# facebookresearch/hanabi_SAD

Measured on AMD Instinct MI355X. Metric: hanabi_env_steps_per_sec, higher is better.
Workload: dtype u32

## Files before the change

### hanabi_sad_amd/csrc/hsad_env.hip

```cpp

#include <hip/hip_runtime.h>

#include <cstdarg>
#include <cstdlib>
#include <cstdio>
#include <cstring>
#include <new>
#include <string>
#include <vector>

#include "hsad.h"
#include "hsad_deal_fast.h"
#include "hsad_obs_row.h"
#include "hsad_planes.h"

namespace {

constexpr int kWave = 64;
constexpr int kMtN = 624;
constexpr int kMtM = 397;

struct EnvParams {
  static constexpr bool kScripted = false;
  int G, Gpad, P, H, A, F, F0, LAL, OB, OD, OL, OK, DECKW;
  int max_len, sad, shuffle_color, bomb, kmode, n_eps, track_dh, npl;
  int nthreads;
  int gpw;
  int obs_words, legal_words, own_words, win_w;
  int win_words;
  int seed0, deal_mode, nt_stores;
  int g_begin, g_count;
  unsigned long long policy_seed;
  int n_iter;
  int delta;
  int compact;
  int stagger_ticks;
  int stagger_mode;
  int64_t* a_out;
  int64_t* g_out;
  uint32_t* planes;
  uint32_t* mt;
  const float* eps_list;
  uint8_t* deck_hist;
  uint32_t* err;
  uint32_t* act_count;
  unsigned long long* legal_bits;
  float* priv_s;
  float* legal;
  float* own;
  float* eps;
  unsigned long long* priv_bits;
  unsigned long long* legal_out;
  unsigned long long* own_bits;
  unsigned short* priv16;
  int pw64, ld16, obs_f32;
  unsigned dbg_units_hi;
  float* reward;
  uint8_t* terminal;
  unsigned long long* dbg;
  int dbg_iters;
  unsigned dbg_units_lo;
  unsigned long long* phase;
  int part, n_part, lock_ticks;
  unsigned long long launch_tag, first_tag;
  unsigned long long* pace;
  unsigned long long pace_base;
  unsigned long long pace_inv_q32;
  int pace_blocks;
  int pace_l0_q8, pace_cap_ticks;
  int nC, nR, max_info, max_life, deck_max, variant;
  unsigned long long deck_full;
};

struct DealScript {
  uint8_t* cards;
  int32_t* count;
};
struct ScriptedParams : EnvParams {
  static constexpr bool kScripted = true;
  DealScript sc;
};

constexpr uint32_t kIdentityPerm = (0u) | (1u << 3) | (2u << 6) | (3u << 9) | (4u << 12);
constexpr uint32_t kIdentityPermBoth = kIdentityPerm | (kIdentityPerm << 15);
__host__ __device__ constexpr uint64_t full_deck_bits() {
  uint64_t d = 0;
  for (int c = 0; c < 5; ++c) {
    const int cnt[5] = {3, 2, 2, 2, 1};
    for (int r = 0; r < 5; ++r) d |= (uint64_t)cnt[r] << (2 * (c * 5 + r));
  }
  return d;
}

__host__ __device__ constexpr uint64_t deck_bits(int C, int R) {
  uint64_t d = 0;
  for (int c = 0; c < C; ++c)
    for (int r = 0; r < R; ++r) d |= (uint64_t)(r == 0 ? 3 : (r == R - 1 ? 1 : 2)) << (2 * (c * 5 + r));
  return d;
}

struct Rules {
  int C, R, MI, ML;
  int deck;
  uint64_t full;
  uint32_t cmask, rmask;
  int CR, KS, DW;
};
struct FullRules {
  static constexpr int C = 5, R = 5, MI = 8, ML = 3, deck = 50;
  static constexpr uint64_t full = full_deck_bits();
  static constexpr uint32_t cmask = 31u, rmask = 31u;
  static constexpr int CR = 25, KS = 35, DW = 10;
};
template <bool V>
struct RulesOf {
  static __device__ __forceinline__ FullRules make(const EnvParams&) { return FullRules{}; }
};
template <>
struct RulesOf<true> {
  static __device__ __forceinline__ Rules make(const EnvParams& ep) {
    const int C = ep.nC, R = ep.nR;
    return Rules{C, R, ep.max_info, ep.max_life, ep.deck_max, ep.deck_full, (1u << C) - 1u, (1u << R) - 1u, C * R,
                 C * R + C + R, R == 1 ? 3 : 2 * R};
  }
};

constexpr uint32_t kMtUpper = 0x80000000u, kMtLower = 0x7fffffffu, kMtMag = 0x9908b0dfu;

__device__ __forceinline__ uint32_t mt_temper(uint32_t x) {
  x ^= x >> 11;
  x ^= (x << 7) & 0x9d2c5680u;
  x ^= (x << 15) & 0xefc60000u;
  x ^= x >> 18;
  return x;
// ... 903 lines not shown
  return df_select(mask, h % (uint32_t)__popcll(mask));
}
__device__ __forceinline__ uint64_t policy_key(uint64_t seed, uint64_t game, int p, int stream) {
  return mix64(seed ^ mix64(game * 0xD1342543DE82EF95ull + (uint64_t)(p * 2 + stream)));
}
__device__ __forceinline__ int policy_pick_keyed(uint64_t key, uint64_t counter, uint64_t mask, int nbits) {
  const uint32_t h = (uint32_t)(mix64(key + counter) >> 32);
  return df_select(mask, h % (uint32_t)__popcll(mask), nbits);
}

constexpr int kEnvThreads = 4 * kWave;

__device__ __forceinline__ void stream_rows(const EnvParams& ep, const uint32_t* s_obs, const uint32_t* s_legal, const uint32_t* s_own,
                                            int g0, int ng, int P, int H, int t, int n) {
  const size_t PF = (size_t)P * ep.F, PA = (size_t)P * ep.A, PO = (size_t)P * 3 * H;
  if (!ep.obs_f32) {
  } else if (ep.nt_stores) {
    stream_bits_f32_aligned<true>(s_obs, ep.priv_s + (size_t)g0 * PF, (uint32_t)(ng * PF), t, n);
  } else {
    stream_bits_f32_aligned<false>(s_obs, ep.priv_s + (size_t)g0 * PF, (uint32_t)(ng * PF), t, n);
  }
  stream_rows_packed(ep, s_obs, 0, ng * P, (size_t)g0 * P, t, n);
  stream_bits_f32_aligned<false>(s_legal, ep.legal + (size_t)g0 * PA, (uint32_t)(ng * PA), t, n);
  stream_bits_f32_aligned<false>(s_own, ep.own + (size_t)g0 * PO, (uint32_t)(ng * PO), t, n);
}

__device__ __forceinline__ unsigned stream_rows_delta(const EnvParams& ep, const uint32_t* s_obs, uint32_t* s_old, bool all,
                                                      const uint32_t* s_legal, const uint32_t* s_own, int g0, int ng, int P, int H,
                                                      int t, int n, bool count, int compact, unsigned& units) {
  const size_t PF = (size_t)P * ep.F, PA = (size_t)P * ep.A, PO = (size_t)P * 3 * H;
  unsigned stored = 0;
  bool by_lines = true;
  if (!ep.obs_f32) {
  } else if (compact && !all) {
    by_lines = false;
    float* out = ep.priv_s + (size_t)g0 * PF;
    if (compact == 2) {
      if (ep.nt_stores) {
        stored = stream_bits_f32_compact<true, 16>(s_obs, s_old, out, (uint32_t)(ng * PF), t, units);
      } else {
        stored = stream_bits_f32_compact<false, 16>(s_obs, s_old, out, (uint32_t)(ng * PF), t, units);
      }
    } else if (ep.nt_stores) {
      stored = stream_bits_f32_compact<true, 32>(s_obs, s_old, out, (uint32_t)(ng * PF), t, units);
    } else {
      stored = stream_bits_f32_compact<false, 32>(s_obs, s_old, out, (uint32_t)(ng * PF), t, units);
    }
  } else if (ep.nt_stores) {
    stored = stream_bits_f32_delta<true>(s_obs, s_old, all, ep.priv_s + (size_t)g0 * PF, (uint32_t)(ng * PF), t, n, count);
  } else {
    stored = stream_bits_f32_delta<false>(s_obs, s_old, all, ep.priv_s + (size_t)g0 * PF, (uint32_t)(ng * PF), t, n, count);
  }
  if (by_lines) units = stored;
  stream_rows_packed(ep, s_obs, 0, ng * P, (size_t)g0 * P, t, n);
  stream_bits_f32_aligned<false>(s_legal, ep.legal + (size_t)g0 * PA, (uint32_t)(ng * PA), t, n);
  stream_bits_f32_aligned<false>(s_own, ep.own + (size_t)g0 * PO, (uint32_t)(ng * PO), t, n);
  return stored;
}

__device__ __forceinline__ void clear_words(uint32_t* p, int nz, int t, int n) {
  uint4* z4 = reinterpret_cast<uint4*>(p);
  for (int k = t; k < (nz >> 2); k += n) z4[k] = make_uint4(0u, 0u, 0u, 0u);
  for (int k = (nz & ~3) + t; k < nz; k += n) p[k] = 0u;
}

__device__ __forceinline__ void clear_rows(const EnvParams& ep, uint32_t* s_obs, int t, int n) {
  const int nz = ep.obs_words + ep.legal_words + ep.own_words;
  uint4* z4 = reinterpret_cast<uint4*>(s_obs);
  for (int k = t; k < (nz >> 2); k += n) z4[k] = make_uint4(0u, 0u, 0u, 0u);
  for (int k = (nz & ~3) + t; k < nz; k += n) s_obs[k] = 0u;
}

struct LogicCarry {
  uint32_t* counter;
  const uint32_t* s_lmask;
  const uint64_t* pkey;
};
template <int TP, int TH>
constexpr bool kPolicyKeys = (TP == 2 && TH == 5);
template <int N>
__device__ __forceinline__ uint64_t carried_key(const uint64_t* k, int i) {
  uint64_t v = k[0];
#pragma unroll
  for (int j = 1; j < N; ++j) v = (i == j) ? k[j] : v;
  return v;
}
typedef __attribute__((address_space(3))) const uint32_t* LdsWordPtr;

template <int MODE, int TP, int TH, bool V = false, class EP = EnvParams, bool CARRY = false>
__device__ __forceinline__ void env_logic(const EP& ep, const int64_t* __restrict__ a_in, const int64_t* __restrict__ g_in,
                                          uint32_t* s_st, uint32_t* s_win, const float* s_eps, const int lane, const int g,
                                          const bool active, const bool do_reset, Rng& rng, uint32_t& greedy_rec, float& reward,
                                          bool& term, const int dbg_it = 0, const LogicCarry carry = {nullptr, nullptr, nullptr}) {
  const int P = TP ? TP : ep.P, H = TH ? TH : ep.H;
  const auto ru = RulesOf<V>::make(ep);
  if (MODE == 0 || MODE == 3) {
    const int W = ep.win_w;
    constexpr int kWmin = (TP && !V) ? (2 * TP * TH + TP + 2 < 64 ? 2 * TP * TH + TP + 2 : 64) : 0;
    constexpr int kWmax = (TP && !V) ? (kWmin + 1 + 2 * (TP - 1) < 64 ? kWmin + 1 + 2 * (TP - 1) : 64) : 64;
    constexpr int kNB = kWmax <= 32 ? kWmax : 32;
    uint32_t* winA = s_win + lane;
    uint32_t* winB = s_win + (W <= 32 ? 0 : (W + 1) * kWave) + lane;
    const uint32_t wbase = rng.spos;
    if (do_reset) {
      if (kWmax <= 32 || (kWmin <= 32 && W <= 32)) {
        const uint32_t* pw = rng.mt + wbase;
// ... 375 lines not shown
        __builtin_amdgcn_s_sleep(8);
      }
    }
  }
  STAMP_START();
  const uint32_t misc0 = ep.planes[(size_t)PL_MISC * ep.Gpad + g];
  bool active;
  const bool needs_reset = valid && (!((misc0 >> 15) & 1u) || ((misc0 >> 14) & 1u));
  if (MODE == 0) {
    active = needs_reset;
    if (__ballot(active) == 0ull) return;
  } else {
    active = valid;
  }
  const bool do_reset = (MODE == 0 || MODE == 3) && needs_reset;
  if (wave == 0) {
    for (int pl0 = 0; pl0 < ep.npl; pl0 += 8) {
      uint32_t v[8];
#pragma unroll
      for (int j = 0; j < 8; ++j) v[j] = ep.planes[(size_t)min(pl0 + j, ep.npl - 1) * ep.Gpad + g];
#pragma unroll
      for (int j = 0; j < 8; ++j)
        if (pl0 + j < ep.npl) ST(pl0 + j) = v[j];
    }
  } else {
    const int zt = tid - kWave, zn = nthreads - kWave;
    clear_rows(ep, s_obs, zt, zn);
    if (MODE == 0 || MODE == 3)
      for (int k = zt; k < min(ep.n_eps, 128); k += zn) s_eps[k] = ep.eps_list[k];
  }
  __syncthreads();
  STAMP(1);

  Rng rng;
  rng.mt = ep.mt + (size_t)g * kMtN;
  rng.draws = ST(PL_DRAWS);
  rng.la0 = ST(PL_LA0);
  rng.la1 = ST(PL_LA1);
  rng.la_n = (int)((ST(PL_MISC) >> 22) & 3u);
  rng.spos = (rng.draws + (uint32_t)rng.la_n) % (uint32_t)kMtN;
  rng.win = nullptr;
  rng.w_c = rng.w_n = 0;
  uint32_t greedy_rec = 0;
  float reward = 0.f;
  bool term = false;

  if (wave == 0) {
    env_logic<MODE, TP, TH, V>(ep, a_in, g_in, s_st, s_win, s_eps, lane, g, active, do_reset, rng, greedy_rec, reward, term, dbg_it);
    s_grec[lane] = greedy_rec;
  }
  __syncthreads();
  STAMP(2);

  Refill rf;
  refill_issue(rf, rng, active && wave == 0);
  if (active) build_rows<TP, TH, V>(ep, s_st, lane, g, s_obs, s_legal, s_own, s_grec[lane], wave, nwaves);
  STAMP(3);
  if (active && wave == 0) {
    refill_finish(rf, rng);
    ST(PL_DRAWS) = rng.draws;
    ST(PL_LA0) = rng.la0;
    ST(PL_LA1) = rng.la1;
    ST(PL_MISC) = (ST(PL_MISC) & ~(3u << 22)) | ((uint32_t)rng.la_n << 22);
    for (int pl = 0; pl < ep.npl; ++pl) ep.planes[(size_t)pl * ep.Gpad + g] = ST(pl);
  }
  __syncthreads();
  STAMP(4);

  const size_t PF = (size_t)P * ep.F, PA = (size_t)P * ep.A, PO = (size_t)P * 3 * H;
  if (MODE >= 1) {
    stream_rows(ep, s_obs, s_legal, s_own, g0, ng, P, H, tid, nthreads);
    if (valid && wave == 0) {
      for (int p = 0; p < P; ++p) ep.eps[(size_t)g * P + p] = __uint_as_float(ST(PLEPS(p)));
      ep.reward[g] = reward;
      ep.terminal[g] = term ? 1 : 0;
    }
    if (ep.kmode == 1) {
      __syncthreads();
      if (wave == 0) v0_fixup<V>(ep, s_st, s_obs, __ballot(valid), g0, lane);
    }
  } else {
    if (wave != 0) return;
    uint64_t todo = __ballot(active);
    const uint64_t todo_all = todo;
    while (todo) {
      const int lg = __builtin_ctzll(todo);
      todo &= todo - 1;
      if (ep.obs_f32) stream_bits_f32(s_obs, (uint32_t)(lg * PF), ep.priv_s + (size_t)(g0 + lg) * PF, (uint32_t)PF, lane);
      stream_rows_packed(ep, s_obs, lg * P, P, (size_t)(g0 + lg) * P, lane, kWave);
      stream_bits_f32(s_legal, (uint32_t)(lg * PA), ep.legal + (size_t)(g0 + lg) * PA, (uint32_t)PA, lane);
      stream_bits_f32(s_own, (uint32_t)(lg * PO), ep.own + (size_t)(g0 + lg) * PO, (uint32_t)PO, lane);
    }
    if (active)
      for (int p = 0; p < P; ++p) ep.eps[(size_t)g * P + p] = __uint_as_float(ST(PLEPS(p)));
    if (ep.kmode == 1) {
      __syncthreads();
      v0_fixup<V>(ep, s_st, s_obs, todo_all, g0, lane);
    }
  }
  STAMP(5);
}

template <int MODE, int TP, int TH, bool V = false>
__global__ __launch_bounds__(kEnvThreads) void env_kernel(EnvParams ep, const int64_t* __restrict__ a_in,
                                                          const int64_t* __restrict__ g_in) {
  env_body<MODE, TP, TH, V>(ep, a_in, g_in);
}

template <int TP, int TH, bool V = false>
__global__ __launch_bounds__(kEnvThreads) void env_step_scripted_kernel(ScriptedParams ep, const int64_t* __restrict__ a_in,
                                                                        const int64_t* __restrict__ g_in) {
  env_body<1, TP, TH, V>(ep, a_in, g_in);
}

__device__ __forceinline__ void rollout_stagger(const EnvParams& ep) {
  if (ep.stagger_ticks > 0) {
    unsigned k = blockIdx.x & 7u;
    if (ep.stagger_mode == 1) k = ((blockIdx.x >> 3) >> 5) & 3u;
    else if (ep.stagger_mode == 2) k = (blockIdx.x >> 3) & 3u;
    else if (ep.stagger_mode == 3) {
      unsigned hw;
      asm volatile("s_getreg_b32 %0, hwreg(HW_REG_HW_ID)" : "=s"(hw));
      k = (hw & 15u) >> 1;
    }
// ... 1 lines not shown
    while (wall_clock64() - t_in < wait) __builtin_amdgcn_s_sleep(16);
  }
}

__device__ __forceinline__ unsigned pace_delay(const EnvParams& ep, unsigned long long s, int iter, unsigned t_own) {
  const long long num = (long long)iter * ep.pace_blocks - (long long)(s - ep.pace_base);
  const long long span = (long long)ep.n_iter * ep.pace_blocks;
  if (num < -span || num > span) return 0u;
  const int over_q8 = (int)((num * (long long)ep.pace_inv_q32) >> 24) - ep.pace_l0_q8;
  if (over_q8 <= 0) return 0u;
  t_own = min(t_own, 1u << 20);
  const unsigned long long d = ((unsigned long long)(unsigned)over_q8 * t_own) >> 8;
  return (unsigned)min(d, (unsigned long long)min(t_own >> 1, (unsigned)ep.pace_cap_ticks));
}

__device__ __forceinline__ unsigned long long pace_count(const EnvParams& ep) {
  int z = 0;
  unsigned long long one = 1ull;
  asm volatile("" : "+v"(z), "+v"(one));
  return __hip_atomic_fetch_add(ep.pace + z, one, __ATOMIC_RELAXED, __HIP_MEMORY_SCOPE_AGENT);
}

__device__ __forceinline__ void pace_sleep(unsigned ticks) {
  const unsigned long long t_in = wall_clock64();
  while (wall_clock64() - t_in < (unsigned long long)ticks) __builtin_amdgcn_s_sleep(16);
}

template <int TP, int TH, bool V = false>
__global__ __launch_bounds__(kEnvThreads) __attribute__((amdgpu_waves_per_eu(2, 2))) void env_rollout_kernel(EnvParams ep) {
  rollout_stagger(ep);
  unsigned long long pace_s = 0ull;
  unsigned pace_t0 = (unsigned)wall_clock64();
  const bool paced = ep.pace && ep.g_begin + (int)blockIdx.x * ep.gpw < ep.G;
#pragma clang loop unroll(disable)
  for (int iter = 0; iter < ep.n_iter; ++iter) {
    if (iter) __syncthreads();
    if (paced) {
      const unsigned now = (unsigned)wall_clock64(), t_own = now - pace_t0;
      pace_t0 = now;
      if (threadIdx.x == 0) {
        if (iter > 0) {
          const unsigned d = pace_delay(ep, pace_s, iter - 1, t_own);
          if (d) pace_sleep(d);
        }
        pace_s = pace_count(ep);
      }
    }
    int zero = 0;
    asm volatile("" : "+s"(zero));
    env_body<3, TP, TH, V>(ep, nullptr, nullptr, zero, iter);
  }
}

#ifdef HSAD_ENV_ROWBUILD_SCATTER
template <int TP, int TH>
constexpr bool kRowBuildFixed = false;
#else
template <int TP, int TH>
constexpr bool kRowBuildFixed = TP > 0 && TH > 0;
#endif

__device__ __forceinline__ unsigned wave_sum(unsigned v) {
  for (int o = kWave / 2; o > 0; o >>= 1) v += (unsigned)__shfl_xor((int)v, o, kWave);
  return v;
}

constexpr int kChainIn = 2, kChainOut = 4;
constexpr int kPrioShift = 3;
__device__ __forceinline__ uint4* chain_slice(const EnvParams& ep) {
  return reinterpret_cast<uint4*>(reinterpret_cast<uint32_t*>(ep.phase) + (size_t)blockIdx.x * ep.obs_words);
}

template <int TP, int TH>
__global__ __launch_bounds__(kEnvThreads) __attribute__((amdgpu_waves_per_eu(2, 2))) void env_rollout_pipe_kernel(EnvParams ep) {
  if constexpr (kRowBuildFixed<TP, TH>) asm volatile("" ::: "v175");
  rollout_stagger(ep);
  extern __shared__ __attribute__((aligned(16))) uint32_t smem[];
  uint32_t* s_st = smem;
  uint32_t* s_obs = s_st + ep.npl * kWave;
  uint32_t* s_legal = s_obs + ep.obs_words;
  uint32_t* s_own = s_legal + ep.legal_words;
  uint32_t* s_win = s_own + ep.own_words;
  uint32_t* s_grec = s_win + ep.win_words * kWave;
  float* s_eps = reinterpret_cast<float*>(s_grec + kWave);
  uint32_t* s_pace = s_grec + kWave + 128;
#define S_OBS1(z) (delta ? s_pace + 4 + (z) : s_obs)
  const int delta = ep.delta & 7;

  const int tid = threadIdx.x;
  const int lane = tid & (kWave - 1);
  const int wave = tid >> 6;
  const int g0 = ep.g_begin + blockIdx.x * ep.gpw;
  const int ng = min(ep.gpw, ep.G - g0);
  if (ng <= 0) return;
  const int P = TP ? TP : ep.P, H = TH ? TH : ep.H;

  unsigned hw_self;
  asm volatile("s_getreg_b32 %0, hwreg(HW_REG_HW_ID)" : "=s"(hw_self));
  const int prio_mode = (ep.delta >> kPrioShift) & 3;
  const int prio_role = (prio_mode & 2) ? 2 * __builtin_amdgcn_readfirstlane(wave) : 0;
  const int prio_alt = prio_mode & 1, prio_slot = (int)(hw_self & 15u);

  uint32_t act_counter = 0u;
  uint64_t pkey[kPolicyKeys<TP, TH> ? 2 * TP : 1] = {};
  if (wave == 0) {
    const int g = g0 + lane;
    if (lane < ng) {
      act_counter = ep.act_count[g];
      if constexpr (kPolicyKeys<TP, TH>) {
#pragma unroll
        for (int k = 0; k < 2 * TP; ++k) pkey[k] = policy_key(ep.policy_seed, (uint64_t)g, k >> 1, k & 1);
      }
      for (int p = 0; p < P; ++p) {
        const uint64_t lm = ep.legal_bits[(size_t)g * P + p];
        s_win[(2 * p) * kWave + lane] = (uint32_t)lm;
        s_win[(2 * p + 1) * kWave + lane] = (uint32_t)(lm >> 32);
      }
    }
    for (int pl0 = 0; pl0 < ep.npl; pl0 += 8) {
      uint32_t v[8];
// ... 356 lines not shown
  size_t d_records_cap;
  uint8_t* d_log_script;
  int32_t* d_log_count;
  int64_t* d_log_a;
};

namespace {

typedef void (*EnvKernelFn)(EnvParams, const int64_t*, const int64_t*);

EnvKernelFn pick_env_kernel(int mode, int P, int H, bool variant) {
  if (variant) {
    switch (mode) {
      case 0: return env_kernel<0, 0, 0, true>;
      case 1: return env_kernel<1, 0, 0, true>;
      case 2: return env_kernel<2, 0, 0, true>;
      default: return env_kernel<3, 0, 0, true>;
    }
  }
#define HSAD_ENV_SPECIALISE(PP, HH)                 \
  if (P == PP && H == HH) {                         \
    switch (mode) {                                 \
      case 0: return env_kernel<0, PP, HH>;         \
      case 1: return env_kernel<1, PP, HH>;         \
      case 2: return env_kernel<2, PP, HH>;         \
      default: return env_kernel<3, PP, HH>;        \
    }                                               \
  }
  HSAD_ENV_SPECIALISE(2, 5)
  HSAD_ENV_SPECIALISE(5, 4)
  HSAD_ENV_SPECIALISE(3, 5)
  HSAD_ENV_SPECIALISE(4, 4)
#undef HSAD_ENV_SPECIALISE
  switch (mode) {
    case 0: return env_kernel<0, 0, 0>;
    case 1: return env_kernel<1, 0, 0>;
    case 2: return env_kernel<2, 0, 0>;
    default: return env_kernel<3, 0, 0>;
  }
}

typedef void (*EnvScriptedStepFn)(ScriptedParams, const int64_t*, const int64_t*);
EnvScriptedStepFn pick_scripted_step_kernel(int P, int H, bool variant) {
  if (variant) return env_step_scripted_kernel<0, 0, true>;
  if (P == 2 && H == 5) return env_step_scripted_kernel<2, 5>;
  if (P == 5 && H == 4) return env_step_scripted_kernel<5, 4>;
  if (P == 3 && H == 5) return env_step_scripted_kernel<3, 5>;
  if (P == 4 && H == 4) return env_step_scripted_kernel<4, 4>;
  return env_step_scripted_kernel<0, 0>;
}

typedef void (*EnvRolloutFn)(EnvParams);
constexpr int kRolloutPrioDefault = 2;
constexpr int kPaceL0Q8 = 0;
constexpr int kPaceCapTicks = 3500;
bool rollout_pipelined(const hsad_env* e) {
  return e->rollout_pipe && e->ep.nthreads == 2 * kWave && e->ep.kmode == 0 && !e->ep.variant;
}

bool rollout_delta_active(const hsad_env* e) {
  return e->rollout_delta && e->delta_fits && rollout_pipelined(e) && e->ep.obs_f32;
}

bool rollout_paced(const hsad_env* e) {
  if (e->rollout_pace >= 0) return e->rollout_pace != 0;
  return !(e->rollout_compact && rollout_delta_active(e));
}

int rollout_chain_mode(const hsad_env* e) {
  return rollout_delta_active(e) && !e->chain_unavailable ? e->rollout_chain : 0;
}

EnvRolloutFn pick_rollout_kernel(int P, int H, bool pipe, bool variant) {
  if (variant) return env_rollout_kernel<0, 0, true>;
#define HSAD_ROLLOUT_SPECIALISE(PP, HH) \
  if (P == PP && H == HH) return pipe ? env_rollout_pipe_kernel<PP, HH> : env_rollout_kernel<PP, HH>;
  HSAD_ROLLOUT_SPECIALISE(2, 5)
  HSAD_ROLLOUT_SPECIALISE(5, 4)
  HSAD_ROLLOUT_SPECIALISE(3, 5)
  HSAD_ROLLOUT_SPECIALISE(4, 4)
#undef HSAD_ROLLOUT_SPECIALISE
  return pipe ? env_rollout_pipe_kernel<0, 0> : env_rollout_kernel<0, 0>;
}

int configure_env_kernels(hsad_env* e) {
  HIP_TRY(hipFuncSetAttribute(reinterpret_cast<const void*>(pick_rollout_kernel(e->ep.P, e->ep.H, false, e->ep.variant != 0)),
                              hipFuncAttributeMaxDynamicSharedMemorySize, (int)e->lds_bytes_reset));
  e->delta_fits = false;
  if (!e->ep.variant) {
    const void* fn = reinterpret_cast<const void*>(pick_rollout_kernel(e->ep.P, e->ep.H, true, false));
    const bool room = e->lds_bytes_delta <= 160 * 1024;
    HIP_TRY(hipFuncSetAttribute(fn, hipFuncAttributeMaxDynamicSharedMemorySize, (int)(room ? e->lds_bytes_delta : e->lds_bytes_reset)));
    if (room) {
      int wg_full = 0, wg_delta = 0;
      HIP_TRY(hipOccupancyMaxActiveBlocksPerMultiprocessor(&wg_full, fn, 2 * kWave, e->lds_bytes_reset));
      HIP_TRY(hipOccupancyMaxActiveBlocksPerMultiprocessor(&wg_delta, fn, 2 * kWave, e->lds_bytes_delta));
      e->delta_fits = wg_delta >= 1 && wg_delta >= wg_full;
    }
  }
  for (int mode = 0; mode < 4; ++mode) {
    const size_t lds = (mode == 1 || mode == 2) ? e->lds_bytes : e->lds_bytes_reset;
    HIP_TRY(hipFuncSetAttribute(reinterpret_cast<const void*>(pick_env_kernel(mode, e->ep.P, e->ep.H, e->ep.variant != 0)),
                                hipFuncAttributeMaxDynamicSharedMemorySize, (int)lds));
  }
  return HSAD_OK;
}

void launch_env(hsad_env* e, int mode, const int64_t* a, const int64_t* g, hipStream_t stream, int g_begin,
                int g_count, uint64_t policy_seed = 0, int64_t* a_out = nullptr, int64_t* g_out = nullptr, int part = -1,
                unsigned long long tag = 0, unsigned long long first_tag = 0, int n_part = 1, int n_iter = 1,
                int chain = 0) {
  size_t lds = (mode == 1 || mode == 2) ? e->lds_bytes : e->lds_bytes_reset;
  EnvParams ep = e->ep;
  ep.delta = mode == 3 && n_iter > 1 && rollout_delta_active(e) ? 1 : 0;
  ep.compact = ep.delta && e->rollout_compact ? (e->rollout_unit == 64 ? 2 : 1) : 0;
  if (ep.delta) lds = e->lds_bytes_delta;
  ep.phase = part >= 0 ? e->d_phase : nullptr;
  ep.part = part < 0 ? 0 : part;
  ep.lock_ticks = (int)(e->stagger_ns / 10);
  ep.launch_tag = tag;
  ep.first_tag = first_tag;
  if (part < 0 && ep.delta && chain && e->d_chain) {
    ep.phase = reinterpret_cast<unsigned long long*>(e->d_chain);
    ep.delta |= chain;
  }
  if (mode == 3 && n_iter > 1 && rollout_pipelined(e)) ep.delta |= e->rollout_prio << kPrioShift;
  ep.n_part = n_part;
  ep.g_begin = g_begin;
  ep.g_count = g_count;
  ep.policy_seed = policy_seed;
  ep.n_iter = n_iter;
  ep.stagger_ticks = n_iter > 1 ? (int)(e->stagger_ns / 10) : 0;
  static const int stagger_mode = getenv("HSAD_ENV_STAGGER_MODE") ? atoi(getenv("HSAD_ENV_STAGGER_MODE")) : 0;
  ep.stagger_mode = stagger_mode;
  ep.a_out = a_out;
  ep.g_out = g_out;
  ep.pace = nullptr;
  if (mode == 3 && n_iter > 1 && rollout_paced(e)) {
    const int g_end = std::min(ep.G, g_begin + g_count);
    const long long blocks = g_end > g_begin ? (g_end - g_begin + ep.gpw - 1) / ep.gpw : 0;
    if (blocks > 0 && blocks * n_iter < (1ll << 29)) {
      ep.pace = e->d_pace;
      ep.pace_base = e->pace_base + (unsigned long long)e->pace_bias;
      ep.pace_blocks = (int)blocks;
      ep.pace_inv_q32 = (1ull << 32) / (unsigned long long)blocks;
      ep.pace_l0_q8 = e->pace_l0_q8;
      ep.pace_cap_ticks = e->pace_cap_ticks;
      e->pace_base += (unsigned long long)(blocks * n_iter);
    }
  }
  if (mode == 3 && n_iter > 1)
    hipLaunchKernelGGL(pick_rollout_kernel(ep.P, ep.H, rollout_pipelined(e), ep.variant != 0), dim3((g_count + ep.gpw - 1) / ep.gpw), dim3(ep.nthreads), lds, stream, ep);
  else if (mode == 1 && e->scripted) {
    ScriptedParams sp;
    static_cast<EnvParams&>(sp) = ep;
    sp.sc = e->script;
    hipLaunchKernelGGL(pick_scripted_step_kernel(ep.P, ep.H, ep.variant != 0), dim3((g_count + ep.gpw - 1) / ep.gpw), dim3(ep.nthreads),
                       lds, stream, sp, a, g);
  }
  else
    hipLaunchKernelGGL(pick_env_kernel(mode, ep.P, ep.H, ep.variant != 0), dim3((g_count + ep.gpw - 1) / ep.gpw), dim3(ep.nthreads), lds,
                       stream, ep, a, g);
}

}

extern "C" {

const char* hsad_last_error(void) { return g_last_error.c_str(); }
int hsad_internal_set_error(int code, const char* msg) {
  g_last_error = msg ? msg : "";
  return code;
}
const char* hsad_version(void) { return "hsad 0.1 gfx950"; }

int hsad_env_create(const hsad_env_config* cfg, hsad_env** out) { return hsad_env_create_rules(cfg, nullptr, out); }

int hsad_env_create_rules(const hsad_env_config* cfg, const hsad_env_rules* rules, hsad_env** out) {
  if (!cfg || !out) return set_error(HSAD_ERR_INVALID, "null argument");
  *out = nullptr;
  const hsad_env_rules full = {5, 5, 8, 3};
  const hsad_env_rules ru = rules ? *rules : full;
  if (ru.colors < 1 || ru.colors > 5) return set_error(HSAD_ERR_INVALID, "colors must be 1..5");
  if (ru.ranks < 1 || ru.ranks > 5) return set_error(HSAD_ERR_INVALID, "ranks must be 1..5");
  if (ru.max_information_tokens < 1 || ru.max_information_tokens > 8)
    return set_error(HSAD_ERR_INVALID, "max_information_tokens must be 1..8");
  if (ru.max_life_tokens < 1 || ru.max_life_tokens > 3) return set_error(HSAD_ERR_INVALID, "max_life_tokens must be 1..3");
  const int Cn = ru.colors, Rn = ru.ranks;
  const int deck_max = Cn * (Rn == 1 ? 3 : 2 * Rn);
  if (cfg->num_games < 1) return set_error(HSAD_ERR_INVALID, "num_games must be >= 1");
  if (cfg->players < 2 || cfg->players > 5) return set_error(HSAD_ERR_INVALID, "players must be 2..5");
  if (cfg->hand_size < 1 || cfg->hand_size > 5) return set_error(HSAD_ERR_INVALID, "hand_size must be 1..5");
  if (cfg->players * cfg->hand_size > deck_max)
    return set_error(HSAD_ERR_INVALID, "players * hand_size (%d) exceeds the deck (%d cards)", cfg->players * cfg->hand_size, deck_max);
  if (cfg->shuffle_obs) return set_error(HSAD_ERR_INVALID, "shuffle_obs is not supported (reference asserts it off)");
  if (cfg->n_eps < 1 || !cfg->eps_list) return set_error(HSAD_ERR_INVALID, "eps_list must hold >= 1 value");
  if (cfg->knowledge_mode != 0 && cfg->knowledge_mode != 1) return set_error(HSAD_ERR_INVALID, "knowledge_mode 0|1");
  if (cfg->max_len > 255) return set_error(HSAD_ERR_INVALID, "max_len must be <= 255");
  if (cfg->games_per_workgroup != 0 && cfg->games_per_workgroup != 32 && cfg->games_per_workgroup != 64)
    return set_error(HSAD_ERR_INVALID, "games_per_workgroup must be 0 (auto), 32 or 64");
  HIP_TRY(hipSetDevice(cfg->device));

  hsad_env* e = new (std::nothrow) hsad_env();
  if (!e) return set_error(HSAD_ERR_NOMEM, "host allocation failed");
// ... 254 lines not shown
}

int hsad_env_step(hsad_env* e, const int64_t* a, const int64_t* greedy_a, void* stream) {
  if (!e) return set_error(HSAD_ERR_INVALID, "null env");
  if (!e->bound) return set_error(HSAD_ERR_STATE, "hsad_env_bind_outputs must be called first");
  if (!a) return set_error(HSAD_ERR_INVALID, "action tensor is null");
  if (e->ep.sad && !greedy_a) return set_error(HSAD_ERR_INVALID, "sad=1 requires greedy_a");
  launch_env(e, 1, a, greedy_a, (hipStream_t)stream, 0, e->ep.Gpad);
  HIP_TRY(hipGetLastError());
  return HSAD_OK;
}

int hsad_env_policy_random(hsad_env* e, uint64_t policy_seed, int64_t* a, int64_t* greedy_a, void* stream) {
  if (!e) return set_error(HSAD_ERR_INVALID, "null env");
  if (!e->bound) return set_error(HSAD_ERR_STATE, "hsad_env_bind_outputs must be called first");
  if (!a) return set_error(HSAD_ERR_INVALID, "action tensor is null");
  EnvParams ep = e->ep;
  ep.g_begin = 0;
  ep.g_count = ep.G;
  hipLaunchKernelGGL(policy_kernel, dim3((ep.G + 255) / 256), dim3(256), 0, (hipStream_t)stream, ep, policy_seed, a,
                     greedy_a);
  HIP_TRY(hipGetLastError());
  return HSAD_OK;
}

int hsad_env_set_partitions(hsad_env* e, int n_part) {
  if (!e) return set_error(HSAD_ERR_INVALID, "null env");
  if (n_part < 1 || n_part > 16) return set_error(HSAD_ERR_INVALID, "n_part must be 1..16");
  const int blocks = e->ep.Gpad / e->ep.gpw;
  if (n_part > blocks) n_part = blocks;
  HIP_TRY(hipSetDevice(e->device));
  for (int k = e->n_part; k < n_part; ++k) {
    HIP_TRY(hipStreamCreateWithFlags(&e->part_stream[k], hipStreamNonBlocking));
    HIP_TRY(hipEventCreate(&e->part_done[k]));
    HIP_TRY(hipEventCreate(&e->part_begin[k]));
  }
  if (!e->fork) HIP_TRY(hipEventCreateWithFlags(&e->fork, hipEventDisableTiming));
  if (n_part > e->n_part) e->n_part = n_part;
  e->n_part_active = n_part;
  return HSAD_OK;
}

int hsad_env_rollout_random(hsad_env* e, int n_iter, uint64_t policy_seed, int64_t* a, int64_t* greedy_a,
                            void* stream) {
  if (!e) return set_error(HSAD_ERR_INVALID, "null env");
  if (!e->bound) return set_error(HSAD_ERR_STATE, "hsad_env_bind_outputs must be called first");
  if (!a) return set_error(HSAD_ERR_INVALID, "action tensor is null");
  if (e->ep.sad && !greedy_a) return set_error(HSAD_ERR_INVALID, "sad=1 requires greedy_a");
  if (e->scripted) return set_error(HSAD_ERR_STATE, "hsad_env_rollout_random: the env holds a deal script (only hsad_env_step deals from it; hsad_env_reset clears it)");
  const int K = e->n_part_active;
  const int blocks = e->ep.Gpad / e->ep.gpw;
  if (e->rollout_chunk > 0) {
    bool chained = rollout_chain_mode(e) != 0 && n_iter > e->rollout_chunk;
    if (chained && !e->d_chain) {
      if (hipMalloc((void**)&e->d_chain, sizeof(uint32_t) * (size_t)blocks * e->ep.obs_words) != hipSuccess) {
        (void)hipGetLastError();
        e->d_chain = nullptr;
        e->chain_unavailable = true;
        chained = false;
      }
    }
    int chain = 0;
    for (int i = 0; i < n_iter; i += e->rollout_chunk) {
      const int n = std::min(e->rollout_chunk, n_iter - i), n_next = std::min(e->rollout_chunk, n_iter - i - n);
      chain = (chain & kChainOut ? kChainIn : 0) | (chained && n > 1 && n_next > 1 ? kChainOut : 0);
      launch_env(e, 3, nullptr, nullptr, (hipStream_t)stream, 0, e->ep.Gpad, policy_seed, a, greedy_a, -1, 0, 0, 1, n, chain);
    }
    HIP_TRY(hipGetLastError());
    return HSAD_OK;
  }
  if (K <= 1) {
    for (int i = 0; i < n_iter; ++i)
      launch_env(e, 3, nullptr, nullptr, (hipStream_t)stream, 0, e->ep.Gpad, policy_seed, a, greedy_a);
    HIP_TRY(hipGetLastError());
    return HSAD_OK;
  }
  HIP_TRY(hipEventRecord(e->fork, (hipStream_t)stream));
  for (int k = 0; k < K; ++k) {
    HIP_TRY(hipStreamWaitEvent(e->part_stream[k], e->fork, 0));
    HIP_TRY(hipEventRecord(e->part_begin[k], e->part_stream[k]));
  }
  e->last_rollout_iters = n_iter;
  e->last_rollout_parts = K;
  if (!e->d_phase) {
    HIP_TRY(hipMalloc((void**)&e->d_phase, sizeof(unsigned long long) * 32));
    HIP_TRY(hipMemset(e->d_phase, 0, sizeof(unsigned long long) * 32));
  }
  const unsigned long long first_tag = e->launch_seq + 1;
  for (int i = 0; i < n_iter; ++i) {
    const unsigned long long tag = ++e->launch_seq;
    for (int k = 0; k < K; ++k) {
      const int b0 = (int)((long long)blocks * k / K), b1 = (int)((long long)blocks * (k + 1) / K);
      if (b1 <= b0) continue;
      launch_env(e, 3, nullptr, nullptr, e->part_stream[k], b0 * e->ep.gpw, (b1 - b0) * e->ep.gpw, policy_seed, a, greedy_a, k, tag,
                 first_tag, K);
    }
  }
  HIP_TRY(hipGetLastError());
  for (int k = 0; k < K; ++k) {
    HIP_TRY(hipEventRecord(e->part_done[k], e->part_stream[k]));
    HIP_TRY(hipStreamWaitEvent((hipStream_t)stream, e->part_done[k], 0));
  }
  return HSAD_OK;
}

int hsad_env_last_rollout_ms(hsad_env* e, float* ms_per_launch, int* n_part) {
  if (!e || !ms_per_launch) return set_error(HSAD_ERR_INVALID, "null argument");
  const int K = e->last_rollout_parts;
  if (n_part) *n_part = K;
  if (K < 2 || e->last_rollout_iters < 1) return set_error(HSAD_ERR_STATE, "no partitioned rollout has run");
  for (int k = 0; k < K; ++k) {
    float ms = 0.f;
    HIP_TRY(hipEventSynchronize(e->part_done[k]));
    HIP_TRY(hipEventElapsedTime(&ms, e->part_begin[k], e->part_done[k]));
    ms_per_launch[k] = ms / (float)e->last_rollout_iters;
  }
  return HSAD_OK;
}

int hsad_env_set_rollout_chunk(hsad_env* e, int iterations_per_launch) {
  if (!e || iterations_per_launch < 0) return set_error(HSAD_ERR_INVALID, "bad argument");
  e->rollout_chunk = iterations_per_launch;
  return HSAD_OK;
}

int hsad_env_set_rollout_pace(hsad_env* e, int on) {
  if (!e) return set_error(HSAD_ERR_INVALID, "null env");
  e->rollout_pace = on != 0;
  return HSAD_OK;
}

int hsad_env_rollout_pace_cap_us(const hsad_env* e) { return e ? e->pace_cap_ticks / 100 : 0; }

int hsad_env_set_rollout_delta(hsad_env* e, int on) {
  if (!e) return set_error(HSAD_ERR_INVALID, "null env");
  e->rollout_delta = on != 0;
  return HSAD_OK;
}

int hsad_env_rollout_delta_active(const hsad_env* e) { return e && rollout_delta_active(e) ? 1 : 0; }

int hsad_env_set_rollout_chain(hsad_env* e, int mode) {
  if (!e || (mode != 0 && mode != 1)) return set_error(HSAD_ERR_INVALID, "the rollout chain mode is 0 or 1");
  e->rollout_chain = mode;
  return HSAD_OK;
}

int hsad_env_rollout_chain_active(const hsad_env* e) { return e ? rollout_chain_mode(e) : 0; }

int hsad_env_set_rollout_prio(hsad_env* e, int mode) {
  if (!e || mode < 0 || mode > 3) return set_error(HSAD_ERR_INVALID, "the rollout priority mode is 0..3");
  e->rollout_prio = mode;
  return HSAD_OK;
}

int hsad_env_rollout_prio(const hsad_env* e) { return e && rollout_pipelined(e) ? e->rollout_prio : 0; }

int hsad_env_set_rollout_compact(hsad_env* e, int on) {
  if (!e) return set_error(HSAD_ERR_INVALID, "null env");
  e->rollout_compact = on != 0;
  return HSAD_OK;
}

int hsad_env_rollout_compact_active(const hsad_env* e) { return e && e->rollout_compact && rollout_delta_active(e) ? 1 : 0; }

int hsad_env_set_rollout_unit(hsad_env* e, int bytes) {
  if (!e || (bytes != 128 && bytes != 64)) return set_error(HSAD_ERR_INVALID, "the rollout unit is 128 or 64 bytes");
  e->rollout_unit = bytes;
  return HSAD_OK;
}

int hsad_env_rollout_unit(const hsad_env* e) { return e ? (hsad_env_rollout_compact_active(e) ? e->rollout_unit : 128) : 0; }

int hsad_env_debug_pace_bias(hsad_env* e, int64_t bias) {
  if (!e) return set_error(HSAD_ERR_INVALID, "null env");
  e->pace_bias = (long long)bias;
  return HSAD_OK;
}

int hsad_env_debug_pace_word(hsad_env* e, int64_t* device_word, int64_t* host_base) {
  if (!e || !device_word || !host_base) return set_error(HSAD_ERR_INVALID, "null argument");
  unsigned long long w = 0;
  HIP_TRY(hipDeviceSynchronize());
  HIP_TRY(hipMemcpy(&w, e->d_pace, sizeof(w), hipMemcpyDeviceToHost));
  *device_word = (int64_t)w;
  *host_base = (int64_t)e->pace_base;
  return HSAD_OK;
}

int hsad_env_set_rollout_stagger(hsad_env* e, int microseconds) {
  if (!e || microseconds < 0) return set_error(HSAD_ERR_INVALID, "bad argument");
  e->stagger_ns = (long long)microseconds * 1000;
  return HSAD_OK;
}

int hsad_env_query(hsad_env* e, int32_t* out, void* stream) {
  if (!e || !out) return set_error(HSAD_ERR_INVALID, "null argument");
  hipLaunchKernelGGL(query_kernel, dim3((e->ep.G + 255) / 256), dim3(256), 0, (hipStream_t)stream, e->ep, out);
  HIP_TRY(hipGetLastError());
  return HSAD_OK;
}

int hsad_env_move_is_legal(hsad_env* e, const int32_t* uid, uint8_t* out, void* stream) {
  if (!e || !uid || !out) return set_error(HSAD_ERR_INVALID, "null argument");
  hipLaunchKernelGGL(legal_query_kernel, dim3((e->ep.G + 255) / 256), dim3(256), 0, (hipStream_t)stream, e->ep, uid,
                     out);
  HIP_TRY(hipGetLastError());
  return HSAD_OK;
}

int hsad_env_deck_history(hsad_env* e, uint8_t* out, int32_t* count, void* stream) {
  if (!e || !out || !count) return set_error(HSAD_ERR_INVALID, "null argument");
  hipLaunchKernelGGL(deck_history_kernel, dim3((e->ep.G + 255) / 256), dim3(256), 0, (hipStream_t)stream, e->ep, out,
                     count);
  HIP_TRY(hipGetLastError());
  return HSAD_OK;
}

int hsad_env_export_state(hsad_env* e, int32_t* out, void* stream) {
  if (!e || !out) return set_error(HSAD_ERR_INVALID, "null argument");
  hipLaunchKernelGGL(export_state_kernel, dim3((e->ep.G + 255) / 256), dim3(256), 0, (hipStream_t)stream, e->ep, out,
                     hsad_env_state_words(e));
  HIP_TRY(hipGetLastError());
  return HSAD_OK;
}

int hsad_env_debug_timing(hsad_env* e, uint64_t* buf) {
  if (!e) return set_error(HSAD_ERR_INVALID, "null env");
  e->ep.dbg = reinterpret_cast<unsigned long long*>(buf);
  e->ep.dbg_iters = 0;
  return HSAD_OK;
}

int hsad_env_debug_trace(hsad_env* e, uint64_t* buf, int n_iters) {
  if (!e || (buf && n_iters < 1)) return set_error(HSAD_ERR_INVALID, "bad argument");
  e->ep.dbg = reinterpret_cast<unsigned long long*>(buf);
  e->ep.dbg_iters = buf ? n_iters : 0;
  return HSAD_OK;
}

int hsad_env_debug_units(hsad_env* e, uint64_t* buf) {
  if (!e) return set_error(HSAD_ERR_INVALID, "null env");
  e->ep.dbg_units_lo = (unsigned)(reinterpret_cast<uint64_t>(buf) & 0xffffffffull);
  e->ep.dbg_units_hi = (unsigned)(reinterpret_cast<uint64_t>(buf) >> 32);
  return HSAD_OK;
}

int64_t hsad_env_rollout_lds_bytes(const hsad_env* e) {
  return e ? (int64_t)(rollout_delta_active(e) ? e->lds_bytes_delta : e->lds_bytes_reset) : 0;
}

int hsad_env_rollout_resident_workgroups(const hsad_env* e) {
  if (!e) return 0;
  const void* fn = reinterpret_cast<const void*>(pick_rollout_kernel(e->ep.P, e->ep.H, rollout_pipelined(e), e->ep.variant != 0));
  int n = 0;
  if (hipOccupancyMaxActiveBlocksPerMultiprocessor(&n, fn, e->ep.nthreads, (size_t)hsad_env_rollout_lds_bytes(e)) != hipSuccess) return -1;
  return n;
}

int hsad_env_error_count(hsad_env* e, int32_t* count, int32_t* first_game, int32_t* first_code) {
  if (!e || !count) return set_error(HSAD_ERR_INVALID, "null argument");
  uint32_t h[4] = {0, 0, 0, 0};
  HIP_TRY(hipDeviceSynchronize());
  HIP_TRY(hipMemcpy(h, e->ep.err, 16, hipMemcpyDeviceToHost));
  *count = (int32_t)h[0];
  if (first_game) *first_game = (int32_t)h[1];
  if (first_code) *first_code = (int32_t)h[2];
  if (h[0]) HIP_TRY(hipMemset(e->ep.err, 0, 16));
  return HSAD_OK;
}

}

#include "hsad_env_search.inc"

#include "hsad_env_belief.inc"

#include "hsad_env_position.inc"

#include "hsad_env_rulebot.inc"

#include "hsad_env_record.inc"
```

Measured before the change: 3.036 billion.

## Add delta-streamed observation rollout kernel for the non-pipelined path

Adds a new rollout kernel for the single (non-pipelined) path. It keeps the previous iteration's observation rows in a per-workgroup global buffer, stages them into the window LDS region, and writes only the float observation lines that changed. This targets the cost of rewriting the full unrolled f32 observation tensor every step. In exchange it adds an extra global read and write of the packed rows each iteration. It depends on rollout_delta being enabled with the pipelined mode off, so it may not run by default.

Result: slower. 2.348 billion (-22.7%).

```diff
diff --git a/hanabi_sad_amd/csrc/hsad_env.hip b/hanabi_sad_amd/csrc/hsad_env.hip
--- a/hanabi_sad_amd/csrc/hsad_env.hip
+++ b/hanabi_sad_amd/csrc/hsad_env.hip
@@ -13,6 +13,7 @@
 #include "hsad_deal_fast.h"
 #include "hsad_obs_row.h"
 #include "hsad_planes.h"
+#include "hsad_rollout_select.h"
 
 namespace {
 
@@ -80,6 +81,14 @@
   static constexpr bool kScripted = true;
   DealScript sc;
 };
+struct DeltaParams : EnvParams {
+  uint32_t* prev;
+  int chain_in;
+};
+template <class EP>
+constexpr bool kDeltaStream = false;
+template <>
+constexpr bool kDeltaStream<DeltaParams> = true;
 
 constexpr uint32_t kIdentityPerm = (0u) | (1u << 3) | (2u << 6) | (3u << 9) | (4u << 12);
 constexpr uint32_t kIdentityPermBoth = kIdentityPerm | (kIdentityPerm << 15);
@@ -1089,6 +1098,63 @@
     stored = stream_bits_f32_delta<false>(s_obs, s_old, all, ep.priv_s + (size_t)g0 * PF, (uint32_t)(ng * PF), t, n, count);
   }
   if (by_lines) units = stored;
+  stream_rows_packed(ep, s_obs, 0, ng * P, (size_t)g0 * P, t, n);
+  stream_bits_f32_aligned<false>(s_legal, ep.legal + (size_t)g0 * PA, (uint32_t)(ng * PA), t, n);
+  stream_bits_f32_aligned<false>(s_own, ep.own + (size_t)g0 * PO, (uint32_t)(ng * PO), t, n);
+  return stored;
+}
+
+__device__ __forceinline__ unsigned wave_sum(unsigned v) {
+  for (int o = kWave / 2; o > 0; o >>= 1) v += (unsigned)__shfl_xor((int)v, o, kWave);
+  return v;
+}
+
+__device__ __forceinline__ void prev_rows_fetch(const uint32_t* slice, uint32_t* s_prev, int nw4, int t, int n) {
+  const uint4* src = reinterpret_cast<const uint4*>(slice);
+  uint4* dst = reinterpret_cast<uint4*>(s_prev);
+  for (int k0 = t; k0 < nw4; k0 += 8 * n) {
+    uint4 v[8];
+#pragma unroll
+    for (int j = 0; j < 8; ++j) v[j] = src[min(k0 + j * n, nw4 - 1)];
+#pragma unroll
+    for (int j = 0; j < 8; ++j)
+      if (k0 + j * n < nw4) dst[k0 + j * n] = v[j];
+  }
+}
+
+__device__ __forceinline__ unsigned stream_rows_prev(const DeltaParams& ep, const uint32_t* s_obs, uint32_t* s_prev, bool all,
+                                                     const uint32_t* s_legal, const uint32_t* s_own, int g0, int ng, int P, int H, int t,
+                                                     int n, bool count) {
+  const size_t PF = (size_t)P * ep.F, PA = (size_t)P * ep.A, PO = (size_t)P * 3 * H;
+  uint32_t* slice = ep.prev + (size_t)blockIdx.x * ep.obs_words;
+  float* out = ep.priv_s + (size_t)g0 * PF;
+  const uint32_t nfl = (uint32_t)(ng * PF);
+  const uint4* cur4 = reinterpret_cast<const uint4*>(s_obs);
+  uint4* slice4 = reinterpret_cast<uint4*>(slice);
+  unsigned stored = 0;
+  if (all) {
+    if (ep.nt_stores) stored = stream_bits_f32_delta<true>(s_obs, s_prev, true, out, nfl, t, n, count);
+    else stored = stream_bits_f32_delta<false>(s_obs, s_prev, true, out, nfl, t, n, count);
+    for (int k = t; k < (ep.obs_words >> 2); k += n) slice4[k] = cur4[k];
+  } else {
+    const int lane = t & (kWave - 1), wave = __builtin_amdgcn_readfirstlane(t >> 6), nwaves = n >> 6;
+    const int g_lo = (int)((nfl + 127u) >> 7);
+    const int q4 = (g_lo + nwaves - 1) / nwaves;
+    const int k_begin = wave * q4, k_end = min(k_begin + q4, g_lo);
+    const uint4* old4 = reinterpret_cast<const uint4*>(s_prev);
+    for (int k = k_begin + lane; k < k_end; k += kWave) {
+      const uint4 c = cur4[k], o = old4[k];
+      if (c.x != o.x || c.y != o.y || c.z != o.z || c.w != o.w) slice4[k] = c;
+    }
+    const uint32_t f_begin = (uint32_t)k_begin * 128u, f_end = min((uint32_t)k_end * 128u, nfl);
+    if (f_begin < f_end) {
+      unsigned units = 0;
+      if (ep.nt_stores)
+        stored = stream_bits_f32_compact<true, 32>(s_obs + 4 * k_begin, s_prev + 4 * k_begin, out + f_begin, f_end - f_begin, lane, units);
+      else
+        stored = stream_bits_f32_compact<false, 32>(s_obs + 4 * k_begin, s_prev + 4 * k_begin, out + f_begin, f_end - f_begin, lane, units);
+    }
+  }
   stream_rows_packed(ep, s_obs, 0, ng * P, (size_t)g0 * P, t, n);
   stream_bits_f32_aligned<false>(s_legal, ep.legal + (size_t)g0 * PA, (uint32_t)(ng * PA), t, n);
   stream_bits_f32_aligned<false>(s_own, ep.own + (size_t)g0 * PO, (uint32_t)(ng * PO), t, n);
@@ -1570,6 +1636,11 @@
   __syncthreads();
   STAMP(2);
 
+  bool prev_all = false;
+  if constexpr (kDeltaStream<EP>) {
+    prev_all = dbg_it == 0 && !ep.chain_in;
+    if (!prev_all) prev_rows_fetch(ep.prev + (size_t)blockIdx.x * ep.obs_words, s_win, ep.obs_words >> 2, tid, nthreads);
+  }
   Refill rf;
   refill_issue(rf, rng, active && wave == 0);
   if (active) build_rows<TP, TH, V>(ep, s_st, lane, g, s_obs, s_legal, s_own, s_grec[lane], wave, nwaves);
@@ -1587,7 +1658,21 @@
 
   const size_t PF = (size_t)P * ep.F, PA = (size_t)P * ep.A, PO = (size_t)P * 3 * H;
   if (MODE >= 1) {
-    stream_rows(ep, s_obs, s_legal, s_own, g0, ng, P, H, tid, nthreads);
+    if constexpr (kDeltaStream<EP>) {
+      const bool dbg_lines = ep.dbg && ep.dbg_iters > 0;
+      unsigned stored = stream_rows_prev(ep, s_obs, s_win, prev_all, s_legal, s_own, g0, ng, P, H, tid, nthreads, dbg_lines);
+      if (dbg_lines) {
+        stored = wave_sum(stored);
+        if (lane == 0) {
+          const size_t rec = ((size_t)(ep.g_begin / ep.gpw) + blockIdx.x) * ep.dbg_iters + (size_t)min(dbg_it, ep.dbg_iters - 1);
+          atomicAdd(ep.dbg + rec * 16 + 13, (unsigned long long)stored);
+          unsigned long long* dbg_units = reinterpret_cast<unsigned long long*>(((uint64_t)ep.dbg_units_hi << 32) | ep.dbg_units_lo);
+          if (dbg_units) atomicAdd(dbg_units + rec, (unsigned long long)stored);
+        }
+      }
+    } else {
+      stream_rows(ep, s_obs, s_legal, s_own, g0, ng, P, H, tid, nthreads);
+    }
     if (valid && wave == 0) {
       for (int p = 0; p < P; ++p) ep.eps[(size_t)g * P + p] = __uint_as_float(ST(PLEPS(p)));
       ep.reward[g] = reward;
@@ -1695,6 +1780,32 @@
   }
 }
 
+template <int TP, int TH>
+__global__ __launch_bounds__(kEnvThreads) __attribute__((amdgpu_waves_per_eu(2, 2))) void env_rollout_delta_kernel(DeltaParams ep) {
+  rollout_stagger(ep);
+  unsigned long long pace_s = 0ull;
+  unsigned pace_t0 = (unsigned)wall_clock64();
+  const bool paced = ep.pace && ep.g_begin + (int)blockIdx.x * ep.gpw < ep.G;
+#pragma clang loop unroll(disable)
+  for (int iter = 0; iter < ep.n_iter; ++iter) {
+    if (iter) __syncthreads();
+    if (paced) {
+      const unsigned now = (unsigned)wall_clock64(), t_own = now - pace_t0;
+      pace_t0 = now;
+      if (threadIdx.x == 0) {
+        if (iter > 0) {
+          const unsigned d = pace_delay(ep, pace_s, iter - 1, t_own);
+          if (d) pace_sleep(d);
+        }
+        pace_s = pace_count(ep);
+      }
+    }
+    int zero = 0;
+    asm volatile("" : "+s"(zero));
+    env_body<3, TP, TH, false, DeltaParams>(ep, nullptr, nullptr, zero, iter);
+  }
+}
+
 #ifdef HSAD_ENV_ROWBUILD_SCATTER
 template <int TP, int TH>
 constexpr bool kRowBuildFixed = false;
@@ -1703,12 +1814,8 @@
 constexpr bool kRowBuildFixed = TP > 0 && TH > 0;
 #endif
 
-__device__ __forceinline__ unsigned wave_sum(unsigned v) {
-  for (int o = kWave / 2; o > 0; o >>= 1) v += (unsigned)__shfl_xor((int)v, o, kWave);
-  return v;
-}
-
 constexpr int kChainIn = 2, kChainOut = 4;
+static_assert(kChainIn == kHsadChainIn && kChainOut == kHsadChainOut, "hsad_rollout_select.h restates the chain flags");
 constexpr int kPrioShift = 3;
 __device__ __forceinline__ uint4* chain_slice(const EnvParams& ep) {
   return reinterpret_cast<uint4*>(reinterpret_cast<uint32_t*>(ep.phase) + (size_t)blockIdx.x * ep.obs_words);
@@ -2171,24 +2278,36 @@
 
 typedef void (*EnvRolloutFn)(EnvParams);
 constexpr int kRolloutPrioDefault = 2;
+constexpr bool kDeltaSinglePaced = false;
 constexpr int kPaceL0Q8 = 0;
 constexpr int kPaceCapTicks = 3500;
 bool rollout_pipelined(const hsad_env* e) {
   return e->rollout_pipe && e->ep.nthreads == 2 * kWave && e->ep.kmode == 0 && !e->ep.variant;
 }
 
-bool rollout_delta_active(const hsad_env* e) {
+bool rollout_delta_pipe(const hsad_env* e) {
   return e->rollout_delta && e->delta_fits && rollout_pipelined(e) && e->ep.obs_f32;
 }
+
+bool rollout_delta_single(const hsad_env* e) {
+  return hsad_rollout_delta_single(e->rollout_delta != 0, rollout_pipelined(e), e->ep.obs_f32 != 0, e->ep.kmode, e->ep.variant != 0,
+                                   e->chain_unavailable, (long long)e->ep.win_words * kWave, e->ep.obs_words);
+}
+
+bool rollout_delta_active(const hsad_env* e) { return rollout_delta_pipe(e) || rollout_delta_single(e); }
 
 bool rollout_paced(const hsad_env* e) {
   if (e->rollout_pace >= 0) return e->rollout_pace != 0;
-  return !(e->rollout_compact && rollout_delta_active(e));
+  if (rollout_delta_single(e)) return kDeltaSinglePaced;
+  return !(e->rollout_compact && rollout_delta_pipe(e));
 }
 
 int rollout_chain_mode(const hsad_env* e) {
   return rollout_delta_active(e) && !e->chain_unavailable ? e->rollout_chain : 0;
 }
+
+typedef void (*EnvRolloutDeltaFn)(DeltaParams);
+EnvRolloutDeltaFn pick_rollout_delta_kernel(int P, int H);
 
 EnvRolloutFn pick_rollout_kernel(int P, int H, bool pipe, bool variant) {
   if (variant) return env_rollout_kernel<0, 0, true>;
@@ -2207,6 +2326,8 @@
                               hipFuncAttributeMaxDynamicSharedMemorySize, (int)e->lds_bytes_reset));
   e->delta_fits = false;
   if (!e->ep.variant) {
+    HIP_TRY(hipFuncSetAttribute(reinterpret_cast<const void*>(pick_rollout_delta_kernel(e->ep.P, e->ep.H)),
+                                hipFuncAttributeMaxDynamicSharedMemorySize, (int)e->lds_bytes_reset));
     const void* fn = reinterpret_cast<const void*>(pick_rollout_kernel(e->ep.P, e->ep.H, true, false));
     const bool room = e->lds_bytes_delta <= 160 * 1024;
     HIP_TRY(hipFuncSetAttribute(fn, hipFuncAttributeMaxDynamicSharedMemorySize, (int)(room ? e->lds_bytes_delta : e->lds_bytes_reset)));
@@ -2231,7 +2352,7 @@
                 int chain = 0) {
   size_t lds = (mode == 1 || mode == 2) ? e->lds_bytes : e->lds_bytes_reset;
   EnvParams ep = e->ep;
-  ep.delta = mode == 3 && n_iter > 1 && rollout_delta_active(e) ? 1 : 0;
+  ep.delta = mode == 3 && n_iter > 1 && rollout_delta_pipe(e) ? 1 : 0;
   ep.compact = ep.delta && e->rollout_compact ? (e->rollout_unit == 64 ? 2 : 1) : 0;
   if (ep.delta) lds = e->lds_bytes_delta;
   ep.phase = part >= 0 ? e->d_phase : nullptr;
@@ -2268,7 +2389,14 @@
       e->pace_base += (unsigned long long)(blocks * n_iter);
     }
   }
-  if (mode == 3 && n_iter > 1)
+  if (mode == 3 && n_iter > 1 && part < 0 && e->d_chain && rollout_delta_single(e)) {
+    DeltaParams dp;
+    static_cast<EnvParams&>(dp) = ep;
+    dp.prev = e->d_chain;
+    dp.chain_in = (chain & kChainIn) ? 1 : 0;
+    hipLaunchKernelGGL(pick_rollout_delta_kernel(ep.P, ep.H), dim3((g_count + ep.gpw - 1) / ep.gpw), dim3(ep.nthreads), lds, stream, dp);
+  }
+  else if (mode == 3 && n_iter > 1)
     hipLaunchKernelGGL(pick_rollout_kernel(ep.P, ep.H, rollout_pipelined(e), ep.variant != 0), dim3((g_count + ep.gpw - 1) / ep.gpw), dim3(ep.nthreads), lds, stream, ep);
   else if (mode == 1 && e->scripted) {
     ScriptedParams sp;
@@ -2629,8 +2757,9 @@
   const int blocks = e->ep.Gpad / e->ep.gpw;
   if (e->rollout_chunk > 0) {
     bool chained = rollout_chain_mode(e) != 0 && n_iter > e->rollout_chunk;
-    if (chained && !e->d_chain) {
-      if (hipMalloc((void**)&e->d_chain, sizeof(uint32_t) * (size_t)blocks * e->ep.obs_words) != hipSuccess) {
+    const bool prev_rows = rollout_delta_single(e) && e->rollout_chunk > 1 && n_iter > 1;
+    if ((chained || prev_rows) && !e->d_chain) {
+      if (hipMalloc((void**)&e->d_chain, hsad_prev_rows_bytes(blocks, e->ep.obs_words)) != hipSuccess) {
         (void)hipGetLastError();
         e->d_chain = nullptr;
         e->chain_unavailable = true;
@@ -2640,7 +2769,7 @@
     int chain = 0;
     for (int i = 0; i < n_iter; i += e->rollout_chunk) {
       const int n = std::min(e->rollout_chunk, n_iter - i), n_next = std::min(e->rollout_chunk, n_iter - i - n);
-      chain = (chain & kChainOut ? kChainIn : 0) | (chained && n > 1 && n_next > 1 ? kChainOut : 0);
+      chain = hsad_chain_flags(chain, chained, n, n_next);
       launch_env(e, 3, nullptr, nullptr, (hipStream_t)stream, 0, e->ep.Gpad, policy_seed, a, greedy_a, -1, 0, 0, 1, n, chain);
     }
     HIP_TRY(hipGetLastError());
@@ -2739,7 +2868,7 @@
   return HSAD_OK;
 }
 
-int hsad_env_rollout_compact_active(const hsad_env* e) { return e && e->rollout_compact && rollout_delta_active(e) ? 1 : 0; }
+int hsad_env_rollout_compact_active(const hsad_env* e) { return e && e->rollout_compact && rollout_delta_pipe(e) ? 1 : 0; }
 
 int hsad_env_set_rollout_unit(hsad_env* e, int bytes) {
   if (!e || (bytes != 128 && bytes != 64)) return set_error(HSAD_ERR_INVALID, "the rollout unit is 128 or 64 bytes");
@@ -2824,12 +2953,14 @@
 }
 
 int64_t hsad_env_rollout_lds_bytes(const hsad_env* e) {
-  return e ? (int64_t)(rollout_delta_active(e) ? e->lds_bytes_delta : e->lds_bytes_reset) : 0;
+  return e ? (int64_t)(rollout_delta_pipe(e) ? e->lds_bytes_delta : e->lds_bytes_reset) : 0;
 }
 
 int hsad_env_rollout_resident_workgroups(const hsad_env* e) {
   if (!e) return 0;
-  const void* fn = reinterpret_cast<const void*>(pick_rollout_kernel(e->ep.P, e->ep.H, rollout_pipelined(e), e->ep.variant != 0));
+  const void* fn = rollout_delta_single(e)
+                       ? reinterpret_cast<const void*>(pick_rollout_delta_kernel(e->ep.P, e->ep.H))
+                       : reinterpret_cast<const void*>(pick_rollout_kernel(e->ep.P, e->ep.H, rollout_pipelined(e), e->ep.variant != 0));
   int n = 0;
   if (hipOccupancyMaxActiveBlocksPerMultiprocessor(&n, fn, e->ep.nthreads, (size_t)hsad_env_rollout_lds_bytes(e)) != hipSuccess) return -1;
   return n;
@@ -2858,3 +2989,13 @@
 #include "hsad_env_rulebot.inc"
 
 #include "hsad_env_record.inc"
+
+namespace {
+EnvRolloutDeltaFn pick_rollout_delta_kernel(int P, int H) {
+  if (P == 2 && H == 5) return env_rollout_delta_kernel<2, 5>;
+  if (P == 5 && H == 4) return env_rollout_delta_kernel<5, 4>;
+  if (P == 3 && H == 5) return env_rollout_delta_kernel<3, 5>;
+  if (P == 4 && H == 4) return env_rollout_delta_kernel<4, 4>;
+  return env_rollout_delta_kernel<0, 0>;
+}
+}
diff --git a/hanabi_sad_amd/csrc/hsad_rollout_select.h b/hanabi_sad_amd/csrc/hsad_rollout_select.h
--- /dev/null
+++ b/hanabi_sad_amd/csrc/hsad_rollout_select.h
@@ -0,0 +1,20 @@
+#pragma once
+
+#include <stddef.h>
+#include <stdint.h>
+
+constexpr int kHsadChainIn = 2, kHsadChainOut = 4;
+
+inline bool hsad_rollout_delta_single(bool delta_on, bool pipelined, bool obs_f32, int kmode, bool variant, bool buffer_unavailable,
+                                      long long window_words, long long obs_words) {
+  return delta_on && !pipelined && obs_f32 && kmode == 0 && !variant && !buffer_unavailable && obs_words > 0 && window_words >= obs_words;
+}
+
+inline size_t hsad_prev_rows_bytes(long long workgroups, long long obs_words) {
+  if (workgroups <= 0 || obs_words <= 0) return 0;
+  return sizeof(uint32_t) * (size_t)workgroups * (size_t)obs_words;
+}
+
+inline int hsad_chain_flags(int before, bool chained, int n, int n_next) {
+  return ((before & kHsadChainOut) ? kHsadChainIn : 0) | (chained && n > 1 && n_next > 1 ? kHsadChainOut : 0);
+}
```
